# ebartrum/lightning_gan_zoo

Hardware: AMD Instinct MI355X
Metric: images/sec (G+D step) at 64x64 bs=128/GPU (higher is better)
Workload: dtype f32; 1 GPU; dc_gan synthetic 64x64 bs=128/GPU, one optimizer cycle of 2 batches (Lightning alternation + toggle), reference optimizer, fp32; key=dc_gan_bs128, global_batch=128, parallelism=dp1, images_counted=2*bs*n_gpus per step (every batch of the cycle)

## Files before the change

lightning_gan_zoo_amd/csrc/gz_igemm2.h:

```cpp
#pragma once
#include "gz_igemm_core.h"

namespace gz {

constexpr int STAGES2 = 3;
constexpr uint32_t SOFF_OOB = 0x80000000u;

template <int WM_, int WN_, int TN_, int OCC_, int TM_ = 4>
struct TileCfg2 {
    static constexpr int WM = WM_, WN = WN_, TM = TM_, TN = TN_, OCC = OCC_;
    static constexpr int BM = WM * TM * 32, BN = WN * TN * 32;
    static_assert(WM * WN == 4, "4 wavefronts per workgroup, one per SIMD");
};

template <int BN>
struct MContigB2 {
    static_assert(BN == 64 || BN == 128 || BN == 256, "piece mapping");
    using Params = typename MContigLoader<BN>::Params;
    static constexpr int LD = BN, ROWS = BK;
    static constexpr int PIECES = BK * BN / 256 / 4;
    static constexpr int RPP = 256 / BN;
    __amdgpu_buffer_rsrc_t rsrc;
    uint32_t voff, ldb;
    int wave;
    __device__ __forceinline__ void init(const Params& p, int tile, int y, int tid) {
        rsrc = make_rsrc(p.base + (long long)y * p.batch_stride, (uint32_t)p.K * p.ld * 4u);
        const int lane = tid & 63;
        wave = __builtin_amdgcn_readfirstlane(tid >> 6);
        const int f = lane * 4, r = f / BN, col = f % BN;
        const int n = tile * BN + col;
        ldb = (uint32_t)p.ld * 4u;
        voff = n < p.MN ? (uint32_t)(r * p.ld + n) * 4u : OOB;
    }
    __device__ __forceinline__ void issue_piece(int kc, float* stage, int p, bool live) {
        const int piece = wave * PIECES + p;
        bload_lds16(rsrc, stage + piece * 256, voff, live ? (uint32_t)(kc * BK + piece * RPP) * ldb : SOFF_OOB);
    }
};

template <int BM>
struct ConvDgA2 {
    static_assert(BM == 256 || BM == 512, "whole 256-pixel pieces per LDS row");
    using Params = typename ConvDgALoader<BM, 4, 4, 2, 1>::Params;
    static constexpr int PPR = BM / 256;
    static constexpr int LD = BM + 4, ROWS = BK / 2, PIECES = 2 * PPR;
    static constexpr int ZERO_COL = BM;
    static constexpr bool ROWSHARE = true;
    __amdgpu_buffer_rsrc_t rsrc;
    uint32_t voff[2 * PPR];
    int wave, K, OHW, shift_half1;
    __device__ __forceinline__ void init(const Params& p, int tile, int phase, int tid) {
        const ConvShape& s = p.s;
        rsrc = make_rsrc(p.y, (uint32_t)s.N * s.K * s.OH * s.OW * 4u);
        const int lane = tid & 63;
        wave = __builtin_amdgcn_readfirstlane(tid >> 6);
        K = s.K; OHW = s.OH * s.OW;
        const int py = phase / 2, px = phase % 2;
        shift_half1 = (px + 1) / 2 - 1;
#pragma unroll
        for (int hb = 0; hb < PPR; ++hb) {
            const uint32_t m = (uint32_t)tile * BM + hb * 256 + lane * 4;
            const bool m_ok = m < (uint32_t)s.N * p.AH * p.AW;
            const uint32_t n = fdiv(m, p.div_ahw);
            const uint32_t pix = m - n * (uint32_t)(p.AH * p.AW);
            const uint32_t a = fdiv(pix, p.div_aw);
            const uint32_t b = pix - a * (uint32_t)p.AW;
#pragma unroll
            for (int ty = 0; ty < 2; ++ty) {
                const int oy = (int)a + (py + 1) / 2 - ty;
                const bool ok = m_ok && (unsigned)oy < (unsigned)s.OH;
                voff[ty * PPR + hb] = ok ? (n * (uint32_t)(s.K * OHW) + (uint32_t)(oy * s.OW) + b) * 4u : OOB;
            }
        }
    }
    __device__ __forceinline__ int frag_shift(int half) const { return half ? shift_half1 : shift_half1 + 1; }
    __device__ __forceinline__ void issue_piece(int kc, float* stage, int p, bool live) {
        const int kol = kc * (BK / 4) + wave;
        bload_lds16(rsrc, stage + (wave * 2 + p / PPR) * LD + (p % PPR) * 256, voff[p],
                    (live && kol < K) ? (uint32_t)kol * (uint32_t)OHW * 4u : SOFF_OOB);
    }
};

template <int BM, int OWC>
struct ConvFwdA2 {
    static_assert(BM == 256 && BM % OWC == 0 && OWC >= 2, "piece mapping");
    using Params = typename ConvFwdALoader<BM, 4, 4, 2, 1>::Params;
    static constexpr int LD = BM, ROWS = BK / 2, PIECES = 2;
    static constexpr int OW_C = OWC;
    static constexpr int EXTRA = (6 * OWC + 4 + 3) & ~3;
    static constexpr bool FWDROWS = true;
    __amdgpu_buffer_rsrc_t rsrc;
    uint32_t voff[2];
    int wave, HW, C;
    __device__ __forceinline__ void init(const Params& p, int tile, int y, int tid) {
        const ConvShape& s = p.s;
        rsrc = make_rsrc(p.x, (uint32_t)(s.N * s.C * s.H * s.W) * 4u);
        const int lane = tid & 63;
        wave = __builtin_amdgcn_readfirstlane(tid >> 6);
        HW = s.H * s.W; C = s.C;
#pragma unroll
        for (int q = 0; q < 2; ++q) {
            const int f = ((wave * 2 + q) * 64 + lane) * 4;
            const int seg = f / (8 * OWC), rem = f - seg * 8 * OWC;
            const int ky = rem / (2 * OWC), col = rem - ky * 2 * OWC;
            const uint32_t m = (uint32_t)tile * BM + seg * OWC;
            const bool m_ok = m < (uint32_t)s.N * s.OH * s.OW;
            const uint32_t n = fdiv(m, p.div_ohw);
            const uint32_t oy = fdiv(m - n * (uint32_t)(s.OH * s.OW), p.div_ow);
            const int iy = (int)oy * 2 - 1 + ky;
            const bool ok = m_ok && (unsigned)iy < (unsigned)s.H;
            voff[q] = ok ? (n * (uint32_t)(s.C * HW) + (uint32_t)(iy * s.W + col)) * 4u : OOB;
        }
    }
    static constexpr int ZERO = ROWS * LD;
    __device__ __forceinline__ void frag(int m_local, int half, int& even, int& odd) const {
        const int seg = m_local / OWC, ox = m_local - seg * OWC;
        const int base = seg * 8 * OWC + 2 * ox - 1 + half;
        even = (half == 0 && ox == 0) ? ZERO : base;
        odd = (half == 1 && ox == OWC - 1) ? ZERO : base + 2;
    }
    __device__ __forceinline__ void issue_piece(int kc, float* stage, int p, bool live) {
        bload_lds16(rsrc, stage + (wave * 2 + p) * 256, voff[p], (live && kc < C) ? (uint32_t)kc * (uint32_t)HW * 4u : SOFF_OOB);
    }
};

template <int BM, int KH, int KW, int S, int P>
struct ConvTapA2 {
    static constexpr bool TAPGATHER = true;
    using Params = typename ConvFwdALoader<BM, KH, KW, S, P>::Params;
    static constexpr int LD = BM, ROWS = BK;
    static constexpr int G = BM / 64;
    static constexpr int PIECES = BK * G / 4;
    __amdgpu_buffer_rsrc_t rsrc;
    uint32_t vbase[G], veff[G];
    int iy0[G], ix0[G];
    int wave, C, H, W, HW, cblocks, last_tap, last_kc, cb;
    uint32_t tap_soff;
    __device__ __forceinline__ void init(const Params& p, int tile, int y, int tid) {
        const ConvShape& s = p.s;
        const uint32_t shift = (uint32_t)(P * s.W + P) * 4u;
        rsrc = make_rsrc(reinterpret_cast<const char*>(p.x) - shift, (uint32_t)s.N * s.C * s.H * s.W * 4u + shift);
        const int lane = tid & 63;
        wave = __builtin_amdgcn_readfirstlane(tid >> 6);
        C = s.C; H = s.H; W = s.W; HW = s.H * s.W;
        cblocks = round_bk(s.C) / BK;
        last_tap = -1; last_kc = -1; cb = 0; tap_soff = 0;
#pragma unroll
        for (int g = 0; g < G; ++g) {
            const uint32_t m = (uint32_t)tile * BM + g * 64 + lane;
            const bool m_ok = m < (uint32_t)s.N * s.OH * s.OW;
            const uint32_t n = fdiv(m, p.div_ohw);
            const uint32_t pix = m - n * (uint32_t)(s.OH * s.OW);
            const uint32_t oy = fdiv(pix, p.div_ow);
            const uint32_t ox = pix - oy * (uint32_t)s.OW;
            iy0[g] = m_ok ? (int)oy * S - P : -(1 << 20);
            ix0[g] = (int)ox * S - P;
            vbase[g] = (n * (uint32_t)(s.C * HW) + (uint32_t)((iy0[g] + P) * W + (ix0[g] + P))) * 4u;
            veff[g] = OOB;
        }
    }
    __device__ __forceinline__ void issue_piece(int kc, float* stage, int p, bool live) {
        if (p == 0) {
            int tap = last_tap;
            if (kc == last_kc + 1 && last_kc >= 0) {
                cb += BK;
                if (cb >= cblocks * BK) { cb = 0; ++tap; }
            } else {
                tap = kc / cblocks;
                cb = (kc - tap * cblocks) * BK;
            }
            last_kc = kc;
            if (tap != last_tap) {
                last_tap = tap;
                const int dy = tap / KW, dx = tap - dy * KW;
                tap_soff = (uint32_t)(dy * W + dx) * 4u;
#pragma unroll
                for (int g = 0; g < G; ++g)
                    veff[g] = ((unsigned)(iy0[g] + dy) < (unsigned)H && (unsigned)(ix0[g] + dx) < (unsigned)W) ? vbase[g] : OOB;
            }
        }
        const int row = wave * 4 + p / G, g = p % G;
        const int c = cb + row;
        bload_lds4(rsrc, stage + row * LD + g * 64, veff[g],
                   (live && c < C) ? (uint32_t)c * (uint32_t)HW * 4u + tap_soff : SOFF_OOB);
    }
};

template <int BM>
struct ConvTapAnyA2 {
    static constexpr bool TAPGATHER = true;
    using Params = typename ConvFwdALoaderTapAny<BM>::Params;
    static constexpr int LD = BM, ROWS = BK;
    static constexpr int G = BM / 64;
    static constexpr int PIECES = BK * G / 4;
    __amdgpu_buffer_rsrc_t rsrc;
    uint32_t vbase[G], veff[G];
    int iy0[G], ix0[G];
    int wave, C, H, W, HW, KW, cblocks, last_tap, last_kc, cb;
    uint32_t tap_soff;
    __device__ __forceinline__ void init(const Params& p, int tile, int y, int tid) {
        const ConvShape& s = p.s;
        const uint32_t shift = (uint32_t)(p.PH * s.W + p.PW) * 4u;
        rsrc = make_rsrc(reinterpret_cast<const char*>(p.x) - shift, (uint32_t)s.N * s.C * s.H * s.W * 4u + shift);
        const int lane = tid & 63;
        wave = __builtin_amdgcn_readfirstlane(tid >> 6);
// ... 369 lines not shown
        }
        const int row = wave * 4 + p / G, g = p % G;
        const int ko = kob + row;
        bload_lds4(rsrc, stage + row * LD + g * 64, veff[g],
                   (live && ko < K) ? (uint32_t)ko * (uint32_t)OSP * 4u + tap_soff : SOFF_OOB);
    }
};

#ifdef GZ2_STAMPS
__device__ unsigned long long gz2_stamps[8192 * 8];
#define GZ2_STAMP(var) const unsigned long long var = __builtin_amdgcn_s_memtime()
#else
#define GZ2_STAMP(var)
#endif

#ifndef GZ2_EXP_NOP
#define GZ2_NOP ""
#else
#define GZ2_NOP "s_nop 1\n\t"
#endif
template <int OFF>
__device__ __forceinline__ float lds_rd(uint32_t byte_addr) {
    float v;
    asm volatile("ds_read_b32 %0, %1 offset:%2" : "=v"(v) : "v"(byte_addr), "n"(OFF) : "memory");
    return v;
}
__device__ __forceinline__ void mfma_row(f32x16 (&c)[4], float a, const float (&b)[4]) {
    asm volatile(GZ2_NOP
                 "v_mfma_f32_32x32x2_f32 %0, %5, %4, %0\n\t"
                 "v_mfma_f32_32x32x2_f32 %1, %6, %4, %1\n\t"
                 "v_mfma_f32_32x32x2_f32 %2, %7, %4, %2\n\t"
                 "v_mfma_f32_32x32x2_f32 %3, %8, %4, %3"
                 : "+a"(c[0]), "+a"(c[1]), "+a"(c[2]), "+a"(c[3])
                 : "v"(a), "v"(b[0]), "v"(b[1]), "v"(b[2]), "v"(b[3]));
}
__device__ __forceinline__ void mfma_row(f32x16 (&c)[2], float a, const float (&b)[2]) {
    asm volatile(GZ2_NOP
                 "v_mfma_f32_32x32x2_f32 %0, %3, %2, %0\n\t"
                 "v_mfma_f32_32x32x2_f32 %1, %4, %2, %1"
                 : "+a"(c[0]), "+a"(c[1])
                 : "v"(a), "v"(b[0]), "v"(b[1]));
}
__device__ __forceinline__ void mfma_row(f32x16 (&c)[1], float a, const float (&b)[1]) {
    asm volatile(GZ2_NOP
                 "v_mfma_f32_32x32x2_f32 %0, %2, %1, %0"
                 : "+a"(c[0])
                 : "v"(a), "v"(b[0]));
}
__device__ __forceinline__ void mfma_one(f32x16& c, float a, float b) {
    asm volatile(GZ2_NOP
                 "v_mfma_f32_32x32x2_f32 %0, %2, %1, %0"
                 : "+a"(c)
                 : "v"(a), "v"(b));
}
__device__ __forceinline__ void mfma_row_mn(f32x16 (&c)[4], float a, const float (&b)[4]) {
    asm volatile(GZ2_NOP
                 "v_mfma_f32_32x32x2_f32 %0, %4, %5, %0\n\t"
                 "v_mfma_f32_32x32x2_f32 %1, %4, %6, %1\n\t"
                 "v_mfma_f32_32x32x2_f32 %2, %4, %7, %2\n\t"
                 "v_mfma_f32_32x32x2_f32 %3, %4, %8, %3"
                 : "+a"(c[0]), "+a"(c[1]), "+a"(c[2]), "+a"(c[3])
                 : "v"(a), "v"(b[0]), "v"(b[1]), "v"(b[2]), "v"(b[3]));
}
__device__ __forceinline__ void mfma_row_mn(f32x16 (&c)[2], float a, const float (&b)[2]) {
    asm volatile(GZ2_NOP
                 "v_mfma_f32_32x32x2_f32 %0, %2, %3, %0\n\t"
                 "v_mfma_f32_32x32x2_f32 %1, %2, %4, %1"
                 : "+a"(c[0]), "+a"(c[1])
                 : "v"(a), "v"(b[0]), "v"(b[1]));
}
__device__ __forceinline__ void lgkm_done(float (&a)[4], float (&b)[4]) {
    asm volatile("s_waitcnt lgkmcnt(0)" : "+v"(a[0]), "+v"(a[1]), "+v"(a[2]), "+v"(a[3]), "+v"(b[0]), "+v"(b[1]), "+v"(b[2]), "+v"(b[3]));
}
__device__ __forceinline__ void lgkm_done(float (&a)[4], float (&b)[2]) {
    asm volatile("s_waitcnt lgkmcnt(0)" : "+v"(a[0]), "+v"(a[1]), "+v"(a[2]), "+v"(a[3]), "+v"(b[0]), "+v"(b[1]));
}
__device__ __forceinline__ void lgkm_done(float (&a)[2], float (&b)[4]) {
    asm volatile("s_waitcnt lgkmcnt(0)" : "+v"(a[0]), "+v"(a[1]), "+v"(b[0]), "+v"(b[1]), "+v"(b[2]), "+v"(b[3]));
}
__device__ __forceinline__ void lgkm_done(float (&a)[4], float (&b)[1]) {
    asm volatile("s_waitcnt lgkmcnt(0)" : "+v"(a[0]), "+v"(a[1]), "+v"(a[2]), "+v"(a[3]), "+v"(b[0]));
}

template <class AL, class = void>
struct a_extra_of { static constexpr int value = 0; };
template <class AL>
struct a_extra_of<AL, std::void_t<decltype(AL::EXTRA)>> { static constexpr int value = AL::EXTRA; };
template <class AL>
constexpr int igemm2_a_extra() { return a_extra_of<AL>::value; }
template <class AL, class = void>
struct fwd_ow_of { static constexpr int value = 1; };
template <class AL>
struct fwd_ow_of<AL, std::void_t<decltype(AL::OW_C)>> { static constexpr int value = AL::OW_C; };
template <class AL>
constexpr int fwd_ow() { return fwd_ow_of<AL>::value; }

template <class AL>
constexpr int mode_count_of() {
    if constexpr (is_dualmode<AL>::value) return AL::MODES;
    else return 1;
}
template <class AL>
constexpr bool mode_plain_of(int m, int S) {
    if constexpr (is_dualmode<AL>::value) return AL::step_plain(m, S);
    else return false;
}
template <class AL>
constexpr unsigned mode_mask_of(int m, int S) {
    if constexpr (is_dualmode<AL>::value) return AL::step_mask(m, S);
    else return 0xFu;
}
template <class AL>
constexpr int ksteps_of() {
    if constexpr (is_dualmode<AL>::value) return AL::KSTEPS;
    else return BK / 2;
}
template <class AL>
constexpr int step_arow_of(int m, int S) {
    if constexpr (is_dualmode<AL>::value) return AL::step_arow(m, S);
    else return S;
}
template <class AL>
constexpr int step_brow_of(int m, int S) {
    if constexpr (is_dualmode<AL>::value) return AL::step_brow(m, S);
    else return 2 * S;
}

template <class Cfg, class AL, class BL, int KG>
constexpr int igemm2_ring_floats() {
    return ((STAGES2 * (AL::ROWS * AL::LD + igemm2_a_extra<AL>() + BL::ROWS * BL::LD) + 63) / 64) * 64;
}

template <class Cfg, class AL, class BL, class Epi, int KG = 1>
__global__ __launch_bounds__(NT * KG, KG == 1 ? Cfg::OCC : 2) void igemm2_kernel(typename AL::Params pa, typename BL::Params pb,
                                                                              typename Epi::Params pe, GridMap gm) {
    constexpr int LDA = AL::LD, LDB = BL::LD;
    constexpr int TM = Cfg::TM, TN = Cfg::TN;
    static_assert((TM == 4 || (TM == 2 && is_dualmode<AL>::value)) && (TN == 1 || TN == 2 || TN == 4),
                  "fragment registers of the hand-ordered k-step");
    static_assert(KG == 1 || (KG == 2 && TN <= 2), "two wave groups: the parked accumulators must fit the LDS");
    constexpr bool RS = is_rowshare<AL>::value;
    constexpr bool FR = is_fwdrows<AL>::value;
    constexpr bool DM = is_dualmode<AL>::value;
    static_assert(!DM || (RS && KG == 1 && (TN == 2 || TN == 4)), "multi-mode: row-shared loader, phases in the accumulator blocks");
    constexpr int A_EXTRA = igemm2_a_extra<AL>();
    constexpr int A_ELEMS = AL::ROWS * LDA + A_EXTRA, B_ELEMS = BL::ROWS * LDB;
    constexpr int STAGE = A_ELEMS + B_ELEMS;
    constexpr int PAD = 16;
    extern __shared__ __attribute__((aligned(16))) float smem2[];
    const int kg = KG == 1 ? 0 : __builtin_amdgcn_readfirstlane((int)threadIdx.x >> 8);
    float* const ring = smem2 + PAD + kg * igemm2_ring_floats<Cfg, AL, BL, KG>();
    GZ2_STAMP(st0);
#ifdef GZ2_STAMPS
    const unsigned long long sr0 = __builtin_amdgcn_s_memrealtime();
    unsigned long long st1 = st0, st2 = st0;
#endif

    const int tid = KG == 1 ? (int)threadIdx.x : ((int)threadIdx.x & (NT - 1));
    const int nwg = gridDim.x;
    int bid = blockIdx.x;
    if (gm.stagger > 0 && bid < 512 && blockIdx.z == 0) {
        const unsigned hw = __builtin_amdgcn_s_getreg(((4 - 1) << 11) | (16 << 6) | 4);
        if (hw & 1u) {
            const unsigned long long t_end = __builtin_amdgcn_s_memtime() + (unsigned long long)gm.stagger;
            while (__builtin_amdgcn_s_memtime() < t_end) __builtin_amdgcn_s_sleep(64);
        }
    }
    int y;
    if (gm.var_chunks) {
        const int tiles = gm.tiles_m * gm.tiles_n;
        y = gm.phase_order[bid / tiles];
        bid %= tiles;
    } else {
        if (!gm.no_swizzle) {
            const int q = nwg >> 3, rr = nwg & 7, x = bid & 7, i = bid >> 3;
            bid = (x < rr ? x * (q + 1) : rr * (q + 1) + (x - rr) * q) + i;
        }
        y = bid % gm.ny;
        bid /= gm.ny;
    }
    const int tile_n = bid % gm.tiles_n;
    const int tile_m = bid / gm.tiles_n;
    const int z = blockIdx.z;
    const int kcA = z * gm.chunks_per_split;
    const int kcB = min(gm.var_chunks ? gm.phase_chunks[y] : gm.chunks, kcA + gm.chunks_per_split);
    if (gm.slab && gm.var_chunks && kcA >= kcB) return;
    int kc0 = kcA, kc1 = kcB, kend = kcB;
    if constexpr (KG == 2) {
        const int h = (kcB - kcA + 1) >> 1;
        kc0 = kcA + kg * h;
        kend = kc0 + h;
        kc1 = min(kcB, kend);
    }

    AL al;
    BL bl;
    al.init(pa, tile_m, y, tid);
    bl.init(pb, tile_n, y, tid);

    f32x16 acc[TM][TN];
#pragma unroll
    for (int i = 0; i < TM; ++i)
#pragma unroll
        for (int j = 0; j < TN; ++j)
#pragma unroll
            for (int r = 0; r < 16; ++r) acc[i][j][r] = 0.f;

    const int lane = tid & 63, wave = __builtin_amdgcn_readfirstlane(tid >> 6);
    const int wm = wave / Cfg::WN, wn = wave % Cfg::WN;
    const int half = lane >> 5, l32 = lane & 31;
    const uint32_t lds0 = (uint32_t)(uintptr_t)(__attribute__((address_space(3))) float*)ring;
    uint32_t a_addr[TM];
#pragma unroll
    for (int i = 0; i < TM; ++i)
        a_addr[i] = lds0 + (uint32_t)(B_ELEMS + half * (RS ? 0 : LDA) + wm * TM * 32 + i * 32 + l32) * 4u;
    if constexpr (RS) {
        const int sh = al.frag_shift(half);
#pragma unroll
        for (int i = 0; i < TM; ++i) {
            const int b = (tile_m * Cfg::BM + wm * TM * 32 + i * 32 + l32) % pa.AW;
            const bool zero = (sh < 0 && b == 0) || (sh > 0 && b == pa.AW - 1);
            a_addr[i] = zero ? lds0 + (uint32_t)(B_ELEMS + AL::ZERO_COL) * 4u : a_addr[i] + (uint32_t)(sh * 4);
        }
        if (tid < STAGES2 * AL::ROWS * 4) {
            const int st = tid / (AL::ROWS * 4), q = tid % (AL::ROWS * 4);
            ring[st * STAGE + B_ELEMS + (q >> 2) * LDA + AL::ZERO_COL + (q & 3)] = 0.f;
        }
    }
    uint32_t a_addrB[TM];
    if constexpr (DM) {
#pragma unroll
        for (int i = 0; i < TM; ++i) {
            const int b = (tile_m * Cfg::BM + wm * TM * 32 + i * 32 + l32) % pa.AW;
            a_addrB[i] = lds0 + (uint32_t)(B_ELEMS + half * LDA + (b == 0 ? AL::ZERO_COL : wm * TM * 32 + i * 32 + l32 - 1)) * 4u;
        }
    }
    uint32_t a_odd[TM];
    if constexpr (FR) {
#pragma unroll
        for (int i = 0; i < TM; ++i) {
            int e, o;
            al.frag(wm * TM * 32 + i * 32 + l32, half, e, o);
            a_addr[i] = lds0 + (uint32_t)(B_ELEMS + e) * 4u;
            a_odd[i] = lds0 + (uint32_t)(B_ELEMS + o) * 4u;
        }
        for (int q = tid; q < STAGES2 * A_EXTRA; q += NT)
            ring[(q / A_EXTRA) * STAGE + B_ELEMS + AL::ZERO + q % A_EXTRA] = 0.f;
    }
    const uint32_t b_addr = lds0 + (uint32_t)(half * LDB + wn * TN * 32 + l32) * 4u;

    constexpr int NPA = AL::PIECES, NPB = BL::PIECES, NP = NPA + NPB, STEPS = ksteps_of<AL>();
    static_assert(STEPS == 8 || STEPS == 12, "k-steps per chunk");
    constexpr int PPS = (NP + STEPS - 1) / STEPS;
    static_assert(PPS <= 4 && NP < 64, "pieces are spread over the k-step's four MFMA rows; vmcnt is 6 bits");
    auto issue_piece = [&](int kc, int st, int p, bool live) {
#ifdef GZ2_EXP_NODMA
        if (kc >= kc0 + 2) return;
#endif
#ifdef GZ2_EXP_SAMECHUNK
        if (kc >= kc0 + 2) kc = kc0;
#endif
        float* sb = ring + st * STAGE;
        if (p < NPA) al.issue_piece(kc, sb + B_ELEMS, p, live);
        else bl.issue_piece(kc, sb, p - NPA, live);
    };
    auto fetch_m = [&](auto Sc, auto Mc, uint32_t so, float (&af)[TM], float (&bf)[TN]) {
        constexpr int S = decltype(Sc)::value, MD = decltype(Mc)::value;
        constexpr bool PL = mode_plain_of<AL>(MD, S);
        constexpr unsigned MK = mode_mask_of<AL>(MD, S);
        constexpr int AO = LDA * step_arow_of<AL>(MD, S) * 4, BO = step_brow_of<AL>(MD, S) * LDB * 4;
#pragma unroll
        for (int i = 0; i < TM; ++i) af[i] = lds_rd<AO>((PL ? a_addrB[i] : a_addr[i]) + so);
        if constexpr ((MK & 1u) != 0) bf[0] = lds_rd<BO>(b_addr + so);
        if constexpr (TN >= 2 && (MK & 2u) != 0) bf[1] = lds_rd<BO + 128>(b_addr + so);
        if constexpr (TN == 4 && (MK & 4u) != 0) bf[2] = lds_rd<BO + 256>(b_addr + so);
        if constexpr (TN == 4 && (MK & 8u) != 0) bf[3] = lds_rd<BO + 384>(b_addr + so);
    };
    auto fetch_first = [&](int kc, uint32_t so, float (&af)[TM], float (&bf)[TN]) {
        if constexpr (DM) {
            if (al.mode_of(kc) == 0) fetch_m(std::integral_constant<int, 0>{}, std::integral_constant<int, 0>{}, so, af, bf);
            else fetch_m(std::integral_constant<int, 0>{}, std::integral_constant<int, 1>{}, so, af, bf);
        }
    };
    auto fetch = [&](auto Sc, uint32_t so, float (&af)[TM], float (&bf)[TN]) {
        constexpr int S = decltype(Sc)::value;
        constexpr int AO = (RS ? LDA : 2 * LDA) * S * 4, BO = 2 * S * LDB * 4;
#ifdef GZ2_EXP_NOFETCH
        if (so != 0xFFFFFFFFu) return;
#endif
        if constexpr (FR) {
            constexpr int FO = (S >> 1) * 2 * fwd_ow<AL>() * 4;
            af[0] = lds_rd<FO>(((S & 1) ? a_odd[0] : a_addr[0]) + so);
            af[1] = lds_rd<FO>(((S & 1) ? a_odd[1] : a_addr[1]) + so);
            af[2] = lds_rd<FO>(((S & 1) ? a_odd[2] : a_addr[2]) + so);
            af[3] = lds_rd<FO>(((S & 1) ? a_odd[3] : a_addr[3]) + so);
        } else {
            af[0] = lds_rd<AO>(a_addr[0] + so);
            af[1] = lds_rd<AO>(a_addr[1] + so);
            af[2] = lds_rd<AO>(a_addr[2] + so);
            af[3] = lds_rd<AO>(a_addr[3] + so);
        }
        {
        bf[0] = lds_rd<BO>(b_addr + so);
        if constexpr (TN >= 2) bf[1] = lds_rd<BO + 128>(b_addr + so);
        if constexpr (TN == 4) {
            bf[2] = lds_rd<BO + 256>(b_addr + so);
            bf[3] = lds_rd<BO + 384>(b_addr + so);
        }
        }
    };
    auto mask = [&](float (&)[TM]) {};

    if (kcA < kcB) {
#pragma unroll
        for (int p = 0; p < NP; ++p) issue_piece(kc0, 0, p, kc0 < kc1);
#pragma unroll
        for (int p = 0; p < NP; ++p) issue_piece(kc0 + 1, 1, p, kc0 + 1 < kc1);
#ifdef GZ2_EXP_NO_LGKM_PROLOGUE
        asm volatile("s_waitcnt vmcnt(%0)" ::"n"(NP) : "memory");
#else
        asm volatile("s_waitcnt vmcnt(%0) lgkmcnt(0)" ::"n"(NP) : "memory");
#endif
        __builtin_amdgcn_s_barrier();
#ifdef GZ2_STAMPS
        st1 = __builtin_amdgcn_s_memtime();
#endif
        float af[2][TM], bf[2][TN];
#ifdef GZ2_STEP_STAMPS
        unsigned long long step_cyc[8] = {0, 0, 0, 0, 0, 0, 0, 0}, step_t = __builtin_amdgcn_s_memtime();
#endif
        if constexpr (DM) {
#pragma unroll
            for (int q = 0; q < 2; ++q)
#pragma unroll
                for (int j = 0; j < TN; ++j) bf[q][j] = 0.f;
            fetch_first(kc0, 0u, af[0], bf[0]);
        } else {
            fetch(std::integral_constant<int, 0>{}, 0u, af[0], bf[0]);
        }
        lgkm_done(af[0], bf[0]);
        mask(af[0]);
        int stage = 0;
        auto run_chunks = [&](int k_from, int k_to, auto Mc) {
        for (int kc = k_from; kc < k_to; ++kc) {
            int s1 = stage + 1; if (s1 >= STAGES2) s1 -= STAGES2;
            int s2 = s1 + 1; if (s2 >= STAGES2) s2 -= STAGES2;
            const uint32_t so = (uint32_t)(stage * STAGE * 4), sno = (uint32_t)(s1 * STAGE * 4);
            const bool more = kc + 2 < kc1;
            auto kstep = [&](auto Sc) {
                constexpr int S = decltype(Sc)::value;
                constexpr int MD = decltype(Mc)::value;
                constexpr int c = S & 1, n = c ^ 1;
                auto mfma_row = [&](f32x16 (&cc)[TN], float a, const float (&b)[TN]) {
                    if constexpr (DM) {
                        constexpr unsigned MK = mode_mask_of<AL>(MD, S);
                        if constexpr (MK == (TN == 4 ? 15u : 3u)) gz::mfma_row(cc, a, b);
                        else {
                            if constexpr ((MK & 1u) != 0) gz::mfma_one(cc[0], a, b[0]);
                            if constexpr (TN >= 2 && (MK & 2u) != 0) gz::mfma_one(cc[1], a, b[1]);
                            if constexpr (TN == 4 && (MK & 4u) != 0) gz::mfma_one(cc[2], a, b[2]);
                            if constexpr (TN == 4 && (MK & 8u) != 0) gz::mfma_one(cc[3], a, b[3]);
                        }
                    } else gz::mfma_row(cc, a, b);
                };
                auto fetch_same = [&](auto S2c, uint32_t o, float (&fa)[TM], float (&fb)[TN]) {
                    if constexpr (DM) fetch_m(S2c, Mc, o, fa, fb);
                    else fetch(S2c, o, fa, fb);
                };
                auto pieces = [&](auto Rowc) {
                    constexpr int row = decltype(Rowc)::value;
                    constexpr int r = PPS == 1 ? (row == 1 ? 0 : -1) : row;
                    constexpr int q = S * PPS + r;
                    if constexpr (r >= 0 && r < PPS && q < NP) issue_piece(kc + 2, s2, q, more);
                };
                if constexpr (S + 1 < STEPS) {
                    fetch_same(std::integral_constant<int, S + 1>{}, so, af[n], bf[n]);
                    mfma_row(acc[0], af[c][0], bf[c]);
                    pieces(std::integral_constant<int, 0>{});
                    mfma_row(acc[1], af[c][1], bf[c]);
                    pieces(std::integral_constant<int, 1>{});
                    if constexpr (TM == 4) mfma_row(acc[2], af[c][2], bf[c]);
                    pieces(std::integral_constant<int, 2>{});
                    if constexpr (TM == 4) mfma_row(acc[3], af[c][3], bf[c]);
                    pieces(std::integral_constant<int, 3>{});
                } else {
                    mfma_row(acc[0], af[c][0], bf[c]);
                    pieces(std::integral_constant<int, 0>{});
                    if constexpr (TM == 4) mfma_row(acc[1], af[c][1], bf[c]);
                    pieces(std::integral_constant<int, 1>{});
                    pieces(std::integral_constant<int, 2>{});
                    pieces(std::integral_constant<int, 3>{});
#ifndef GZ2_EXP_NOVMWAIT
                    asm volatile("s_waitcnt vmcnt(%0)" ::"n"(NP) : "memory");
#endif
#ifndef GZ2_EXP_NOBARRIER
                    __builtin_amdgcn_s_barrier();
#endif
                    if constexpr (DM) fetch_first(kc + 1, sno, af[n], bf[n]);
                    else fetch(std::integral_constant<int, 0>{}, sno, af[n], bf[n]);
                    if constexpr (TM == 4) {
                        mfma_row(acc[2], af[c][2], bf[c]);
                        mfma_row(acc[3], af[c][3], bf[c]);
                    } else {
                        mfma_row(acc[1], af[c][1], bf[c]);
                    }
                }
#ifdef GZ2_STEP_STAMPS
                {
                    const unsigned long long t = __builtin_amdgcn_s_memtime();
                    step_cyc[S] += t - step_t;
                    step_t = t;
                }
#endif
                lgkm_done(af[n], bf[n]);
                mask(af[n]);
            };
            kstep(std::integral_constant<int, 0>{});
            kstep(std::integral_constant<int, 1>{});
            kstep(std::integral_constant<int, 2>{});
            kstep(std::integral_constant<int, 3>{});
            kstep(std::integral_constant<int, 4>{});
            kstep(std::integral_constant<int, 5>{});
            kstep(std::integral_constant<int, 6>{});
            kstep(std::integral_constant<int, 7>{});
            if constexpr (STEPS == 12) {
                kstep(std::integral_constant<int, 8>{});
                kstep(std::integral_constant<int, 9>{});
                kstep(std::integral_constant<int, 10>{});
                kstep(std::integral_constant<int, 11>{});
            }
            stage = s1;
        }
        };
        if constexpr (DM) {
            run_chunks(kc0, min(kend, al.bound[0]), std::integral_constant<int, 0>{});
            run_chunks(max(kc0, al.bound[0]), kend, std::integral_constant<int, 1>{});
        } else {
            run_chunks(kc0, kend, std::integral_constant<int, 0>{});
        }
        asm volatile("s_waitcnt vmcnt(0)\n\ts_nop 15\n\ts_nop 15" ::: "memory");
#ifdef GZ2_STAMPS
        st2 = __builtin_amdgcn_s_memtime();
#endif
#ifdef GZ2_STEP_STAMPS
        if (tid == 0 && blockIdx.x < 64)
            for (int q = 0; q < 8; ++q) gz2_stamps[(size_t)(8192 - 64 + blockIdx.x) * 8 + q] = step_cyc[q];
#endif
    }

    if constexpr (KG == 2) {
        __syncthreads();
        float* const park = smem2;
        if (kg == 1) {
#pragma unroll
            for (int i = 0; i < TM; ++i)
#pragma unroll
                for (int j = 0; j < TN; ++j)
#pragma unroll
                    for (int r = 0; r < 16; ++r) park[((i * TN + j) * 16 + r) * NT + tid] = acc[i][j][r];
        }
        __syncthreads();
        if (kg == 1) return;
#pragma unroll
        for (int i = 0; i < TM; ++i)
#pragma unroll
            for (int j = 0; j < TN; ++j)
#pragma unroll
                for (int r = 0; r < 16; ++r) acc[i][j][r] += park[((i * TN + j) * 16 + r) * NT + tid];
    }
#ifdef GZ2_EXP_NOSTORE
    if (acc[0][0][0] == 123456.789f)
#endif
    if (gm.slab)
        store_slab<Epi::SWAP, TM, TN>(gm, acc, tile_m * Cfg::BM + wm * TM * 32, tile_n * Cfg::BN + wn * TN * 32, lane,
                                      gm.var_chunks ? gm.phase_slab0[y] + z : y * (int)gridDim.z + z);
    else
// ... 408 lines not shown
            kstep(std::integral_constant<int, 4>{});
            kstep(std::integral_constant<int, 5>{});
            kstep(std::integral_constant<int, 6>{});
            kstep(std::integral_constant<int, 7>{});
            stage = s1;
        }
        asm volatile("s_waitcnt vmcnt(0)\n\ts_nop 15\n\ts_nop 15" ::: "memory");
    }
    Epi::template store<TM, TN>(pe, acc, tile_m * Cfg::BM + wm * TM * 32, tile_n * Cfg::BN + wn * TN * 32, lane, 0, z);
}

template <class Cfg, class BL>
constexpr size_t igemm2w_lds_bytes() {
    return (size_t)STAGES2 * (WgDyA2<Cfg::BM>::ELEMS + BL::ELEMS) * 4;
}

template <class Cfg, class BL, class Epi>
inline int launch_igemm2w(const Wg2Params& p, const typename Epi::Params& pe, int M, int N, int K, int splits,
                          hipStream_t stream) {
    GridMap gm;
    gm.no_swizzle = knobs().no_xcd_swizzle;
    gm.var_chunks = 0;
    gm.slab = nullptr;
    gm.slab_m = M;
    gm.slab_n = N;
    gm.tiles_m = (M + Cfg::BM - 1) / Cfg::BM;
    gm.tiles_n = (N + Cfg::BN - 1) / Cfg::BN;
    gm.chunks = (K + BK - 1) / BK;
    if (splits < 1) splits = 1;
    gm.chunks_per_split = (gm.chunks + splits - 1) / splits;
    int nz = (gm.chunks + gm.chunks_per_split - 1) / gm.chunks_per_split;
    if (nz < 1) nz = 1;
    gm.ny = 1;
    gm.stagger = 0;
    for (int i = 0; i < 8; ++i) gm.phase_nz[i] = gm.phase_slab0[i] = 0;
    dim3 grid(gm.tiles_m * gm.tiles_n, 1, nz);
    constexpr size_t lds = igemm2w_lds_bytes<Cfg, BL>();
    static_assert(lds <= 80 * 1024, "two workgroups per CU");
    auto kern = igemm2w_kernel<Cfg, BL, Epi>;
    static bool attr_done = false;
    if (!attr_done) {
        if (hipFuncSetAttribute((const void*)kern, hipFuncAttributeMaxDynamicSharedMemorySize, (int)lds) != hipSuccess)
            return launch_status();
        attr_done = true;
    }
    hipLaunchKernelGGL(kern, grid, dim3(NT), lds, stream, p, pe, gm);
    return launch_status();
}

template <class Cfg, class AL, class BL, class Epi>
inline int launch_igemm2r(const typename AL::Params& pa, const typename BL::Params& pb, const typename Epi::Params& pe,
                          int M, int N, int K, int splits, hipStream_t stream) {
    GridMap gm;
    gm.no_swizzle = knobs().no_xcd_swizzle;
    gm.var_chunks = 0;
    gm.slab = nullptr;
    gm.slab_m = M;
    gm.slab_n = N;
    gm.tiles_m = (M + Cfg::BM - 1) / Cfg::BM;
    gm.tiles_n = (N + Cfg::BN - 1) / Cfg::BN;
    gm.chunks = (K + BK - 1) / BK;
    if (splits < 1) splits = 1;
    gm.chunks_per_split = (gm.chunks + splits - 1) / splits;
    int nz = (gm.chunks + gm.chunks_per_split - 1) / gm.chunks_per_split;
    if (nz < 1) nz = 1;
    gm.ny = 1;
    gm.stagger = 0;
    for (int i = 0; i < 8; ++i) gm.phase_nz[i] = gm.phase_slab0[i] = 0;
    dim3 grid(gm.tiles_m * gm.tiles_n, 1, nz);
    constexpr size_t lds = (size_t)2 * BK * (AL::LD + BL::LD) * 4;
    auto kern = igemm2r_kernel<Cfg, AL, BL, Epi>;
    static bool attr_done = false;
    if (!attr_done) {
        if (hipFuncSetAttribute((const void*)kern, hipFuncAttributeMaxDynamicSharedMemorySize, (int)lds) != hipSuccess)
            return launch_status();
        attr_done = true;
    }
    hipLaunchKernelGGL(kern, grid, dim3(NT), lds, stream, pa, pb, pe, gm);
    return launch_status();
}

template <class Cfg, class AL, class BL>
constexpr size_t igemm2_lds_bytes() {
    return (size_t)(STAGES2 * (AL::ROWS * AL::LD + igemm2_a_extra<AL>() + BL::ROWS * BL::LD) + 32) * 4;
}
template <class Cfg, class AL, class BL>
constexpr size_t igemm2_lds_bytes_kg2() {
    const size_t rings = (size_t)(2 * igemm2_ring_floats<Cfg, AL, BL, 2>() + 32) * 4;
    const size_t park = (size_t)Cfg::TM * Cfg::TN * 16 * NT * 4;
    return rings > park ? rings : park;
}

template <class T, class = void>
struct is_tapgather : std::false_type {};
template <class T>
struct is_tapgather<T, std::void_t<decltype(T::TAPGATHER)>> : std::true_type {};
template <class Cfg, class AL>
constexpr bool igemm2_kg2_built() {
    return Cfg::TN <= 2 && Cfg::WM * Cfg::WN == 4 && Cfg::WN == 2 && !is_dualmode<AL>::value &&
           (is_rowshare<AL>::value || is_fwdrows<AL>::value || is_tapgather<AL>::value);
}
inline bool igemm2_use_kg2(long long workgroups, int chunks_per_workgroup) {
    if (knobs().no_kg2) return false;
    return workgroups <= cus() && chunks_per_workgroup >= knobs().kg2_min_chunks;
}

template <class Cfg, class AL, class BL, class Epi>
inline int launch_igemm2(const typename AL::Params& pa, const typename BL::Params& pb, const typename Epi::Params& pe,
                         int M, int N, int K, int ny, int splits, hipStream_t stream, float* slab = nullptr,
                         const int* phase_chunks = nullptr) {
    static_assert(Epi::SWAP, "transposed accumulators (lanes along m)");
    GridMap gm;
    gm.no_swizzle = knobs().no_xcd_swizzle;
    gm.var_chunks = 0;
    if (phase_chunks && ny <= 8) {
        gm.var_chunks = 1;
        for (int i = 0; i < ny; ++i) {
            gm.phase_chunks[i] = phase_chunks[i];
            gm.phase_order[i] = i;
        }
        for (int i = 1; i < ny; ++i)
            for (int j = i; j > 0 && gm.phase_chunks[gm.phase_order[j]] > gm.phase_chunks[gm.phase_order[j - 1]]; --j) {
                int t = gm.phase_order[j];
                gm.phase_order[j] = gm.phase_order[j - 1];
                gm.phase_order[j - 1] = t;
            }
    }
    gm.slab = nullptr;
    gm.slab_m = M;
    gm.slab_n = N;
    gm.tiles_m = (M + Cfg::BM - 1) / Cfg::BM;
    gm.tiles_n = (N + Cfg::BN - 1) / Cfg::BN;
    gm.chunks = (K + BK - 1) / BK;
    if (splits < 1) splits = 1;
    gm.chunks_per_split = (gm.chunks + splits - 1) / splits;
    int nz = (gm.chunks + gm.chunks_per_split - 1) / gm.chunks_per_split;
    if (nz < 1) nz = 1;
    gm.ny = ny;
    dim3 grid(gm.tiles_m * gm.tiles_n * ny, 1, nz);
    const int stagger_pct = knobs().igemm2_stagger;
    gm.stagger = (Cfg::OCC == 2 && nz == 1 && grid.x >= 1536)
                     ? (int)((long long)gm.chunks * 8 * Cfg::TM * Cfg::TN * 64 * 2 * stagger_pct / 100) : 0;
    if (slab && nz > 1) gm.slab = slab;
    SlabMap sm;
    sm.var = gm.slab && gm.var_chunks;
    for (int i = 0, at = 0; i < 8; ++i) {
        int n = (sm.var && i < ny) ? (gm.phase_chunks[i] + gm.chunks_per_split - 1) / gm.chunks_per_split : 0;
        gm.phase_nz[i] = sm.nz[i] = n;
        gm.phase_slab0[i] = sm.slab0[i] = at;
        at += n;
    }
    const size_t lds_extra = (size_t)knobs().igemm2_lds;
    bool launched = false;
    if constexpr (igemm2_kg2_built<Cfg, AL>()) {
        if (igemm2_use_kg2((long long)grid.x * nz, gm.chunks_per_split)) {
            const size_t lds2 = igemm2_lds_bytes_kg2<Cfg, AL, BL>();
            auto kern2 = igemm2_kernel<Cfg, AL, BL, Epi, 2>;
            static bool attr2_done = false;
            if (!attr2_done) {
                if (hipFuncSetAttribute((const void*)kern2, hipFuncAttributeMaxDynamicSharedMemorySize, (int)lds2) != hipSuccess)
                    return launch_status();
                attr2_done = true;
            }
            hipLaunchKernelGGL(kern2, grid, dim3(2 * NT), lds2, stream, pa, pb, pe, gm);
            launched = true;
        }
    }
// ... 25 lines not shown
```

Baseline: 45210 images/s.

## Restructure forward-conv A tile LDS layout and make ring depth configurable

The forward-conv A loader now stores each kernel row (ky) per wave as a contiguous 2*BM+4 row with a shared zero column, replacing the segment-interleaved layout with its separate EXTRA zero pad. Fragment addressing becomes a simple stride of 2*m. It also generalises the DMA ring from a fixed three stages to NST stages, with the prologue, wait counts and prefetch distance all parameterised, though NST defaults to the old value. The layout change is meant to simplify address math and remove the extra pad init, at the cost of more LDS per stage and a changed bank access pattern.

```diff
diff --git a/lightning_gan_zoo_amd/csrc/gz_igemm2.h b/lightning_gan_zoo_amd/csrc/gz_igemm2.h
--- a/lightning_gan_zoo_amd/csrc/gz_igemm2.h
+++ b/lightning_gan_zoo_amd/csrc/gz_igemm2.h
@@ -85,9 +85,8 @@
 struct ConvFwdA2 {
     static_assert(BM == 256 && BM % OWC == 0 && OWC >= 2, "piece mapping");
     using Params = typename ConvFwdALoader<BM, 4, 4, 2, 1>::Params;
-    static constexpr int LD = BM, ROWS = BK / 2, PIECES = 2;
-    static constexpr int OW_C = OWC;
-    static constexpr int EXTRA = (6 * OWC + 4 + 3) & ~3;
+    static constexpr int LD = 2 * BM + 4, ROWS = BK / 4, PIECES = 2;
+    static constexpr int ZERO_COL = 2 * BM;
     static constexpr bool FWDROWS = true;
     __amdgpu_buffer_rsrc_t rsrc;
     uint32_t voff[2];
@@ -100,9 +99,9 @@
         HW = s.H * s.W; C = s.C;
 #pragma unroll
         for (int q = 0; q < 2; ++q) {
-            const int f = ((wave * 2 + q) * 64 + lane) * 4;
-            const int seg = f / (8 * OWC), rem = f - seg * 8 * OWC;
-            const int ky = rem / (2 * OWC), col = rem - ky * 2 * OWC;
+            const int ky = wave;
+            const int f = (q * 64 + lane) * 4;
+            const int seg = f / (2 * OWC), col = f - seg * 2 * OWC;
             const uint32_t m = (uint32_t)tile * BM + seg * OWC;
             const bool m_ok = m < (uint32_t)s.N * s.OH * s.OW;
             const uint32_t n = fdiv(m, p.div_ohw);
@@ -112,15 +111,14 @@
             voff[q] = ok ? (n * (uint32_t)(s.C * HW) + (uint32_t)(iy * s.W + col)) * 4u : OOB;
         }
     }
-    static constexpr int ZERO = ROWS * LD;
     __device__ __forceinline__ void frag(int m_local, int half, int& even, int& odd) const {
-        const int seg = m_local / OWC, ox = m_local - seg * OWC;
-        const int base = seg * 8 * OWC + 2 * ox - 1 + half;
-        even = (half == 0 && ox == 0) ? ZERO : base;
-        odd = (half == 1 && ox == OWC - 1) ? ZERO : base + 2;
+        const int ox = m_local % OWC;
+        const int base = 2 * m_local - 1 + half;
+        even = (half == 0 && ox == 0) ? ZERO_COL : base;
+        odd = (half == 1 && ox == OWC - 1) ? ZERO_COL : base + 2;
     }
     __device__ __forceinline__ void issue_piece(int kc, float* stage, int p, bool live) {
-        bload_lds16(rsrc, stage + (wave * 2 + p) * 256, voff[p], (live && kc < C) ? (uint32_t)kc * (uint32_t)HW * 4u : SOFF_OOB);
+        bload_lds16(rsrc, stage + wave * LD + p * 256, voff[p], (live && kc < C) ? (uint32_t)kc * (uint32_t)HW * 4u : SOFF_OOB);
     }
 };
 
@@ -656,19 +654,6 @@
     asm volatile("s_waitcnt lgkmcnt(0)" : "+v"(a[0]), "+v"(a[1]), "+v"(a[2]), "+v"(a[3]), "+v"(b[0]));
 }
 
-template <class AL, class = void>
-struct a_extra_of { static constexpr int value = 0; };
-template <class AL>
-struct a_extra_of<AL, std::void_t<decltype(AL::EXTRA)>> { static constexpr int value = AL::EXTRA; };
-template <class AL>
-constexpr int igemm2_a_extra() { return a_extra_of<AL>::value; }
-template <class AL, class = void>
-struct fwd_ow_of { static constexpr int value = 1; };
-template <class AL>
-struct fwd_ow_of<AL, std::void_t<decltype(AL::OW_C)>> { static constexpr int value = AL::OW_C; };
-template <class AL>
-constexpr int fwd_ow() { return fwd_ow_of<AL>::value; }
-
 template <class AL>
 constexpr int mode_count_of() {
     if constexpr (is_dualmode<AL>::value) return AL::MODES;
@@ -700,9 +685,16 @@
     else return 2 * S;
 }
 
+#ifndef GZ2_KG2_STAGES
+#define GZ2_KG2_STAGES STAGES2
+#endif
+template <class Cfg, class AL, int KG>
+constexpr int igemm2_stages() {
+    return (KG == 2 && Cfg::TN == 1 && (is_rowshare<AL>::value || is_fwdrows<AL>::value)) ? GZ2_KG2_STAGES : STAGES2;
+}
 template <class Cfg, class AL, class BL, int KG>
 constexpr int igemm2_ring_floats() {
-    return ((STAGES2 * (AL::ROWS * AL::LD + igemm2_a_extra<AL>() + BL::ROWS * BL::LD) + 63) / 64) * 64;
+    return ((igemm2_stages<Cfg, AL, KG>() * (AL::ROWS * AL::LD + BL::ROWS * BL::LD) + 63) / 64) * 64;
 }
 
 template <class Cfg, class AL, class BL, class Epi, int KG = 1>
@@ -717,8 +709,9 @@
     constexpr bool FR = is_fwdrows<AL>::value;
     constexpr bool DM = is_dualmode<AL>::value;
     static_assert(!DM || (RS && KG == 1 && (TN == 2 || TN == 4)), "multi-mode: row-shared loader, phases in the accumulator blocks");
-    constexpr int A_EXTRA = igemm2_a_extra<AL>();
-    constexpr int A_ELEMS = AL::ROWS * LDA + A_EXTRA, B_ELEMS = BL::ROWS * LDB;
+    constexpr int NST = igemm2_stages<Cfg, AL, KG>();
+    static_assert(NST >= 3 && NST <= 5, "ring depth");
+    constexpr int A_ELEMS = AL::ROWS * LDA, B_ELEMS = BL::ROWS * LDB;
     constexpr int STAGE = A_ELEMS + B_ELEMS;
     constexpr int PAD = 16;
     extern __shared__ __attribute__((aligned(16))) float smem2[];
@@ -796,7 +789,10 @@
             const bool zero = (sh < 0 && b == 0) || (sh > 0 && b == pa.AW - 1);
             a_addr[i] = zero ? lds0 + (uint32_t)(B_ELEMS + AL::ZERO_COL) * 4u : a_addr[i] + (uint32_t)(sh * 4);
         }
-        if (tid < STAGES2 * AL::ROWS * 4) {
+    }
+    if constexpr (RS || FR) {
+        static_assert(NST * AL::ROWS * 4 <= NT, "one thread per pad float");
+        if (tid < NST * AL::ROWS * 4) {
             const int st = tid / (AL::ROWS * 4), q = tid % (AL::ROWS * 4);
             ring[st * STAGE + B_ELEMS + (q >> 2) * LDA + AL::ZERO_COL + (q & 3)] = 0.f;
         }
@@ -818,15 +814,13 @@
             a_addr[i] = lds0 + (uint32_t)(B_ELEMS + e) * 4u;
             a_odd[i] = lds0 + (uint32_t)(B_ELEMS + o) * 4u;
         }
-        for (int q = tid; q < STAGES2 * A_EXTRA; q += NT)
-            ring[(q / A_EXTRA) * STAGE + B_ELEMS + AL::ZERO + q % A_EXTRA] = 0.f;
     }
     const uint32_t b_addr = lds0 + (uint32_t)(half * LDB + wn * TN * 32 + l32) * 4u;
 
     constexpr int NPA = AL::PIECES, NPB = BL::PIECES, NP = NPA + NPB, STEPS = ksteps_of<AL>();
     static_assert(STEPS == 8 || STEPS == 12, "k-steps per chunk");
     constexpr int PPS = (NP + STEPS - 1) / STEPS;
-    static_assert(PPS <= 4 && NP < 64, "pieces are spread over the k-step's four MFMA rows; vmcnt is 6 bits");
+    static_assert(PPS <= 4 && (NST - 1) * NP < 64, "pieces are spread over the k-step's four MFMA rows; vmcnt is 6 bits");
     auto issue_piece = [&](int kc, int st, int p, bool live) {
 #ifdef GZ2_EXP_NODMA
         if (kc >= kc0 + 2) return;
@@ -863,7 +857,7 @@
         if (so != 0xFFFFFFFFu) return;
 #endif
         if constexpr (FR) {
-            constexpr int FO = (S >> 1) * 2 * fwd_ow<AL>() * 4;
+            constexpr int FO = (S >> 1) * LDA * 4;
             af[0] = lds_rd<FO>(((S & 1) ? a_odd[0] : a_addr[0]) + so);
             af[1] = lds_rd<FO>(((S & 1) ? a_odd[1] : a_addr[1]) + so);
             af[2] = lds_rd<FO>(((S & 1) ? a_odd[2] : a_addr[2]) + so);
@@ -887,13 +881,13 @@
 
     if (kcA < kcB) {
 #pragma unroll
-        for (int p = 0; p < NP; ++p) issue_piece(kc0, 0, p, kc0 < kc1);
-#pragma unroll
-        for (int p = 0; p < NP; ++p) issue_piece(kc0 + 1, 1, p, kc0 + 1 < kc1);
+        for (int c = 0; c < NST - 1; ++c)
+#pragma unroll
+            for (int p = 0; p < NP; ++p) issue_piece(kc0 + c, c, p, kc0 + c < kc1);
 #ifdef GZ2_EXP_NO_LGKM_PROLOGUE
-        asm volatile("s_waitcnt vmcnt(%0)" ::"n"(NP) : "memory");
+        asm volatile("s_waitcnt vmcnt(%0)" ::"n"((NST - 2) * NP) : "memory");
 #else
-        asm volatile("s_waitcnt vmcnt(%0) lgkmcnt(0)" ::"n"(NP) : "memory");
+        asm volatile("s_waitcnt vmcnt(%0) lgkmcnt(0)" ::"n"((NST - 2) * NP) : "memory");
 #endif
         __builtin_amdgcn_s_barrier();
 #ifdef GZ2_STAMPS
@@ -917,10 +911,10 @@
         int stage = 0;
         auto run_chunks = [&](int k_from, int k_to, auto Mc) {
         for (int kc = k_from; kc < k_to; ++kc) {
-            int s1 = stage + 1; if (s1 >= STAGES2) s1 -= STAGES2;
-            int s2 = s1 + 1; if (s2 >= STAGES2) s2 -= STAGES2;
+            int s1 = stage + 1; if (s1 >= NST) s1 -= NST;
+            int s2 = stage + NST - 1; if (s2 >= NST) s2 -= NST;
             const uint32_t so = (uint32_t)(stage * STAGE * 4), sno = (uint32_t)(s1 * STAGE * 4);
-            const bool more = kc + 2 < kc1;
+            const bool more = kc + NST - 1 < kc1;
             auto kstep = [&](auto Sc) {
                 constexpr int S = decltype(Sc)::value;
                 constexpr int MD = decltype(Mc)::value;
@@ -945,7 +939,7 @@
                     constexpr int row = decltype(Rowc)::value;
                     constexpr int r = PPS == 1 ? (row == 1 ? 0 : -1) : row;
                     constexpr int q = S * PPS + r;
-                    if constexpr (r >= 0 && r < PPS && q < NP) issue_piece(kc + 2, s2, q, more);
+                    if constexpr (r >= 0 && r < PPS && q < NP) issue_piece(kc + NST - 1, s2, q, more);
                 };
                 if constexpr (S + 1 < STEPS) {
                     fetch_same(std::integral_constant<int, S + 1>{}, so, af[n], bf[n]);
@@ -965,7 +959,7 @@
                     pieces(std::integral_constant<int, 2>{});
                     pieces(std::integral_constant<int, 3>{});
 #ifndef GZ2_EXP_NOVMWAIT
-                    asm volatile("s_waitcnt vmcnt(%0)" ::"n"(NP) : "memory");
+                    asm volatile("s_waitcnt vmcnt(%0)" ::"n"((NST - 2) * NP) : "memory");
 #endif
 #ifndef GZ2_EXP_NOBARRIER
                     __builtin_amdgcn_s_barrier();
@@ -1540,7 +1534,7 @@
 
 template <class Cfg, class AL, class BL>
 constexpr size_t igemm2_lds_bytes() {
-    return (size_t)(STAGES2 * (AL::ROWS * AL::LD + igemm2_a_extra<AL>() + BL::ROWS * BL::LD) + 32) * 4;
+    return (size_t)(STAGES2 * (AL::ROWS * AL::LD + BL::ROWS * BL::LD) + 32) * 4;
 }
 template <class Cfg, class AL, class BL>
 constexpr size_t igemm2_lds_bytes_kg2() {
```

Result: no change. 45560 images/s (median of 6 runs) (+0.8%).
